# yassouali/pytorch-segmentation

Measured on NVIDIA H100. Metric: images/sec DeepLabV3+/ResNet101 513x513 train step (fwd+CE+bwd+SGD), higher is better.
Workload: dtype bf16

## Files before the change

### pytorch-segmentation_b200/csrc/seg_conv_tc.cu

```cuda
#include <cuda.h>
#include <mutex>
#include <stdlib.h>
#include "seg_common.cuh"
#include "seg_ptx.cuh"
#include "seg_sync.cuh"

namespace seg {
namespace tc {

using namespace ptx;

constexpr int BM = 128;
constexpr int BK = 64;
constexpr int A_BYTES = BM * 128;
constexpr int KIND_KK = 0, KIND_KM = 1, KIND_MM = 2;
constexpr int NTHREADS = 384;
constexpr int NCONS = 256;
constexpr int MAXT = 49;

struct TcParams {
  CUtensorMap mapA;
  CUtensorMap mapB;
  int M;
  int Ncols;
  int taps;
  int kchunks;
  int stride;
  int lower_h, lower_w;
  int PQ, Q;
  int x_im2col;
  int brows_per_tap;
  short tap_wt[MAXT];
  short tap_oh[MAXT];
  short tap_ow[MAXT];
  void* out;
  long long ldo;
  int out_dtype;
  float beta;
  const float* bias;
  double* stats;
  unsigned* stat_ticket;
  SyncDesc sync;
  int out_strided, out_H, out_W, osy, osx, opy, opx;
  int kblocks_total, kblocks_per_split;
  float* dw;
  int dw_K, dw_C;
  float* ws;
};

template <int BN>
struct Cfg {
  static constexpr int B_BYTES = BN * 128;
  static constexpr int STAGE_BYTES = A_BYTES + B_BYTES;
  static constexpr int STAGES = BN == 64 ? 6 : (BN == 128 ? 5 : 4);
  static constexpr int STAT_BYTES = 2 * 2 * BN * 4;
  static constexpr int SMEM = STAGES * STAGE_BYTES + STAT_BYTES + 1024  + 256 ;
  static_assert(STAGES * STAGE_BYTES >= BM * BN * 4, "staging tile must fit in the pipeline ring");
  static_assert(SMEM <= 227 * 1024, "shared memory per block");
};

__device__ __forceinline__ void row_to_coords(int m, int PQ, int Q, int stride, int lower_h, int lower_w, int& n, int& h,
                                              int& w) {
  n = m / PQ;
  int rem = m - n * PQ;
  int pp = rem / Q;
  int qq = rem - pp * Q;
  h = lower_h + pp * stride;
  w = lower_w + qq * stride;
}

template <int BN, int TA, int TB>
__device__ __forceinline__ void wgmma_tile(float* acc, uint64_t adesc, uint64_t bdesc, uint32_t accumulate) {
  if constexpr (BN == 64) wgmma_m64n64k16<TA, TB>(acc, adesc, bdesc, accumulate);
  else if constexpr (BN == 128) wgmma_m64n128k16<TA, TB>(acc, adesc, bdesc, accumulate);
  else wgmma_m64n256k16<TA, TB>(acc, adesc, bdesc, accumulate);
}

__device__ __forceinline__ void consumer_sync() { asm volatile("bar.sync 1, 256;" ::: "memory"); }

template <int BN, int KIND>
__global__ void __launch_bounds__(NTHREADS, 1) conv_gemm_tc(const __grid_constant__ TcParams p) {
  using C = Cfg<BN>;
  constexpr int STAGES = C::STAGES;
  extern __shared__ uint8_t smem_raw[];
  const uint32_t raw_addr = smem_u32(smem_raw);
  const uint32_t smem0 = (raw_addr + 1023u) & ~1023u;
  uint8_t* smem_gen = smem_raw + (smem0 - raw_addr);
  float* stat_sm = reinterpret_cast<float*>(smem_gen + STAGES * C::STAGE_BYTES);
  const uint32_t bar0 = smem0 + STAGES * C::STAGE_BYTES + C::STAT_BYTES;
  auto full_bar = [&](int s) { return bar0 + 8u * s; };
  auto empty_bar = [&](int s) { return bar0 + 8u * (STAGES + s); };
  volatile int* flag_sm = reinterpret_cast<volatile int*>(smem_gen + STAGES * C::STAGE_BYTES + C::STAT_BYTES + 8 * 2 * STAGES);

  const int m0 = blockIdx.x * BM;
  const int n0 = blockIdx.y * BN;

  int tap_mm = 0, kb_begin = 0, kb_end = 0, num_iters;
  if (KIND == KIND_MM) {
    tap_mm = blockIdx.z % p.taps;
    const int split = blockIdx.z / p.taps;
    kb_begin = split * p.kblocks_per_split;
    kb_end = min(kb_begin + p.kblocks_per_split, p.kblocks_total);
    num_iters = max(kb_end - kb_begin, 0);
  } else {
    num_iters = p.taps * p.kchunks;
  }

  if (threadIdx.x == 0) {
    prefetch_tmap(&p.mapA);
    prefetch_tmap(&p.mapB);
    for (int s = 0; s < STAGES; ++s) {
      mbar_init(full_bar(s), 1);
      mbar_init(empty_bar(s), 8);
    }
    fence_mbar_init();
  }
  __syncthreads();
  pdl_wait();

  if (threadIdx.x < 128) {
    if (threadIdx.x == 0 && num_iters > 0) {
      if (KIND != KIND_MM) {
        int n_img = 0, h0 = 0, w0 = 0;
        if (p.x_im2col) row_to_coords(m0, p.PQ, p.Q, p.stride, p.lower_h, p.lower_w, n_img, h0, w0);
        int it = 0;
        for (int tap = 0; tap < p.taps; ++tap) {
          const int wtap = p.tap_wt[tap];
          const uint16_t oh = (uint16_t)p.tap_oh[tap], ow = (uint16_t)p.tap_ow[tap];
          for (int kc = 0; kc < p.kchunks; ++kc, ++it) {
            const int st = it % STAGES;
            const uint32_t ph = (it / STAGES) & 1;
            mbar_wait_nocall(empty_bar(st), ph ^ 1u);
            const uint32_t a_dst = smem0 + st * C::STAGE_BYTES;
            const uint32_t b_dst = a_dst + A_BYTES;
            mbar_arrive_expect_tx(full_bar(st), C::STAGE_BYTES);
            if (p.x_im2col)
              tma_load_im2col_4d(a_dst, &p.mapA, full_bar(st), kc * BK, w0, h0, n_img, ow, oh);
            else
              tma_load_2d(a_dst, &p.mapA, full_bar(st), kc * BK, m0);
            if (KIND == KIND_KK) {
              tma_load_2d(b_dst, &p.mapB, full_bar(st), kc * BK, wtap * p.brows_per_tap + n0);
            } else {
#pragma unroll
              for (int j = 0; j < BN / 64; ++j)
                tma_load_2d(b_dst + j * 8192, &p.mapB, full_bar(st), n0 + j * 64, wtap * p.brows_per_tap + kc * BK);
            }
          }
        }
      } else {
        const uint16_t oh = (uint16_t)p.tap_oh[tap_mm], ow = (uint16_t)p.tap_ow[tap_mm];
        int it = 0;
        for (int kb = kb_begin; kb < kb_end; ++kb, ++it) {
          const int st = it % STAGES;
          const uint32_t ph = (it / STAGES) & 1;
          mbar_wait_nocall(empty_bar(st), ph ^ 1u);
          const uint32_t a_dst = smem0 + st * C::STAGE_BYTES;
          const uint32_t b_dst = a_dst + A_BYTES;
          const int pix0 = kb * BK;
          mbar_arrive_expect_tx(full_bar(st), C::STAGE_BYTES);
          tma_load_2d(a_dst, &p.mapA, full_bar(st), m0, pix0);
          tma_load_2d(a_dst + 8192, &p.mapA, full_bar(st), m0 + 64, pix0);
          if (p.x_im2col) {
            int n_img, h0, w0;
            row_to_coords(pix0, p.PQ, p.Q, p.stride, p.lower_h, p.lower_w, n_img, h0, w0);
#pragma unroll
            for (int j = 0; j < BN / 64; ++j)
              tma_load_im2col_4d(b_dst + j * 8192, &p.mapB, full_bar(st), n0 + j * 64, w0, h0, n_img, ow, oh);
          } else {
#pragma unroll
            for (int j = 0; j < BN / 64; ++j) tma_load_2d(b_dst + j * 8192, &p.mapB, full_bar(st), n0 + j * 64, pix0);
          }
        }
      }
    }
    return;
  }

  if (KIND == KIND_MM && num_iters == 0) return;
  const int ctid = threadIdx.x - 128;
  const int cw = ctid >> 7;
  const int warp = (ctid >> 5) & 3, lane = ctid & 31;
  float acc[BN / 2];
#pragma unroll
  for (int i = 0; i < BN / 2; ++i) acc[i] = 0.f;
  {
    constexpr int TA = (KIND == KIND_MM) ? 1 : 0;
    constexpr int TB = (KIND == KIND_KK) ? 0 : 1;
    for (int it = 0; it < num_iters; ++it) {
      const int st = it % STAGES;
      mbar_wait_nocall(full_bar(st), (it / STAGES) & 1);
      const uint32_t a_addr = smem0 + st * C::STAGE_BYTES + cw * 8192;
      const uint32_t b_addr = smem0 + st * C::STAGE_BYTES + A_BYTES;
      const uint64_t adesc0 = make_smem_desc_sw128(a_addr, TA ? 8192 : 16, 1024);
      const uint64_t bdesc0 = make_smem_desc_sw128(b_addr, TB ? 8192 : 16, 1024);
      wgmma_fence();
#pragma unroll
      for (int k = 0; k < BK / 16; ++k) {
        const uint64_t adesc = adesc0 + (uint64_t)(TA ? (k * 2048 >> 4) : (k * 32 >> 4));
        const uint64_t bdesc = bdesc0 + (uint64_t)(TB ? (k * 2048 >> 4) : (k * 32 >> 4));
        wgmma_tile<BN, TA, TB>(acc, adesc, bdesc, 1u);
      }
      wgmma_commit();
      wgmma_wait<1>();
      __syncwarp();
      if (it > 0 && lane == 0) mbar_arrive(empty_bar((it - 1) % STAGES));
    }
    wgmma_wait<0>();
  }
  consumer_sync();

  const bool out_f32 = (KIND == KIND_MM) || p.out_dtype != SEG_DT_BF16;
  const int esize = out_f32 ? 4 : 2;
  const int CPR = BN * esize / 16;
  const int swz = (CPR >= 32 ? 31 : CPR - 1);
  uint8_t* stage = smem_gen;
  const int ncols_tile = min(BN, p.Ncols - n0);
  {
    const int r0 = cw * 64 + warp * 16 + (lane >> 2);
#pragma unroll
    for (int j = 0; j < BN / 8; ++j) {
      const int col = j * 8 + 2 * (lane & 3);
      float b0 = 0.f, b1 = 0.f;
      if (KIND != KIND_MM && p.bias) {
        if (col < ncols_tile) b0 = __ldg(p.bias + n0 + col);
        if (col + 1 < ncols_tile) b1 = __ldg(p.bias + n0 + col + 1);
      }
#pragma unroll
      for (int h = 0; h < 2; ++h) {
        const int r = r0 + 8 * h;
        const float x0 = acc[4 * j + 2 * h] + b0, x1 = acc[4 * j + 2 * h + 1] + b1;
        const int byte = col * esize;
        uint8_t* dst = stage + (size_t)r * (BN * esize) + ((((byte >> 4) ^ (r & swz))) << 4) + (byte & 15);
        if (out_f32)
          *reinterpret_cast<float2*>(dst) = make_float2(x0, x1);
        else
          *reinterpret_cast<__nv_bfloat162*>(dst) = __floats2bfloat162_rn(x0, x1);
      }
    }
  }
  consumer_sync();

  if (KIND == KIND_MM) {
    float* base = p.ws ? p.ws + (size_t)(blockIdx.z / p.taps) * p.taps * p.dw_K * p.dw_C : p.dw;
    for (int idx = ctid; idx < BM * CPR; idx += NCONS) {
      const int tr = idx / CPR, c16 = idx - tr * CPR;
      const int row = m0 + tr, col0 = c16 * 4;
      if (row >= p.M || col0 >= ncols_tile) continue;
      const float4 v = *reinterpret_cast<const float4*>(stage + (size_t)tr * (BN * 4) + ((c16 ^ (tr & swz)) << 4));
      float* dst = base + ((size_t)tap_mm * p.dw_K + row) * p.dw_C + n0 + col0;
      const bool vec = col0 + 4 <= ncols_tile && ((reinterpret_cast<uintptr_t>(dst) & 15) == 0);
      const float a[4] = {v.x, v.y, v.z, v.w};
      if (p.ws) {
        if (vec)
          *reinterpret_cast<float4*>(dst) = v;
        else
          for (int i = 0; i < 4; ++i)
            if (col0 + i < ncols_tile) dst[i] = a[i];
      } else if (vec) {
        asm volatile("red.global.add.v4.f32 [%0], {%1, %2, %3, %4};" ::"l"(dst), "f"(v.x), "f"(v.y), "f"(v.z), "f"(v.w)
                     : "memory");
      } else {
        for (int i = 0; i < 4; ++i)
          if (col0 + i < ncols_tile) atomicAdd(dst + i, a[i]);
      }
    }
    return;
  }

  if (p.stats) {
    constexpr int NG = NCONS / BN, RPG = BM / NG;
    const int c = ctid % BN, g = ctid / BN;
    const int rend = min((g + 1) * RPG, p.M - m0);
    float s1 = 0.f, s2 = 0.f;
    const int byte = c * esize;
    for (int r = g * RPG; r < rend; ++r) {
      const uint8_t* src = stage + (size_t)r * (BN * esize) + ((((byte >> 4) ^ (r & swz))) << 4) + (byte & 15);
      const float x = out_f32 ? *reinterpret_cast<const float*>(src) : bf2f(*reinterpret_cast<const __nv_bfloat16*>(src));
      s1 += x;
      s2 = fmaf(x, x, s2);
    }
    stat_sm[(g * 2 + 0) * BN + c] = s1;
    stat_sm[(g * 2 + 1) * BN + c] = s2;
  }

  {
    const int nchunks = (ncols_tile * esize + 15) >> 4;
    const bool vec_ok = ((p.ldo * esize) & 15) == 0 && ((reinterpret_cast<uintptr_t>(p.out) + (size_t)n0 * esize) & 15) == 0;
    for (int idx = ctid; idx < BM * CPR; idx += NCONS) {
      const int tr = idx / CPR;
      const int c16 = idx - tr * CPR;
      if (c16 >= nchunks) continue;
      const int grow = m0 + tr;
      if (grow >= p.M) continue;
      long long pixel = grow;
      if (p.out_strided) {
        const int n = grow / p.PQ;
        const int rem = grow - n * p.PQ;
        const int i = rem / p.Q, j = rem - i * p.Q;
        pixel = ((long long)n * p.out_H + (i * p.osy + p.opy)) * p.out_W + (j * p.osx + p.opx);
      }
      const uint8_t* src = stage + (size_t)tr * (BN * esize) + ((c16 ^ (tr & swz)) << 4);
      uint8_t* dst = reinterpret_cast<uint8_t*>(p.out) + ((size_t)pixel * p.ldo + n0) * esize + ((size_t)c16 << 4);
      const int first_col = (c16 << 4) / esize;
      const bool full = first_col + 16 / esize <= ncols_tile;
      if (!out_f32) {
        bf16x8 val = *reinterpret_cast<const bf16x8*>(src);
        if (vec_ok && full) {
          if (p.beta != 0.f) {
            float a[8], b[8];
            unpack8(val, a);
            unpack8(*reinterpret_cast<const bf16x8*>(dst), b);
#pragma unroll
            for (int k = 0; k < 8; ++k) a[k] += p.beta * b[k];
            val = pack8(a);
          }
          *reinterpret_cast<bf16x8*>(dst) = val;
        } else {
          float a[8];
          unpack8(val, a);
          __nv_bfloat16* d = reinterpret_cast<__nv_bfloat16*>(dst);
          for (int k = 0; k < 8; ++k)
            if (first_col + k < ncols_tile) {
              float o = a[k];
              if (p.beta != 0.f) o += p.beta * bf2f(d[k]);
              d[k] = f2bf(o);
            }
        }
      } else {
        const float4 val = *reinterpret_cast<const float4*>(src);
        const float a[4] = {val.x, val.y, val.z, val.w};
        float* d = reinterpret_cast<float*>(dst);
        if (vec_ok && full && p.beta == 0.f) {
          *reinterpret_cast<float4*>(d) = val;
        } else {
          for (int k = 0; k < 4; ++k)
            if (first_col + k < ncols_tile) d[k] = (p.beta != 0.f) ? a[k] + p.beta * d[k] : a[k];
        }
      }
    }
  }
  if (num_iters > 0 && ctid == 0) pdl_trigger();

  if (p.stats) {
    constexpr int NG = NCONS / BN;
    consumer_sync();
    for (int c = ctid; c < ncols_tile; c += NCONS) {
      float a = 0.f, b = 0.f;
#pragma unroll
      for (int g = 0; g < NG; ++g) {
        a += stat_sm[(g * 2 + 0) * BN + c];
        b += stat_sm[(g * 2 + 1) * BN + c];
      }
      atomicAdd(p.stats + n0 + c, (double)a);
      atomicAdd(p.stats + p.Ncols + n0 + c, (double)b);
    }
    if (p.sync.world > 0)
      sync_push_when_last<false>(p.sync, p.stats, 2 * p.Ncols, p.stat_ticket, gridDim.x * gridDim.y, ctid, NCONS,
                          [] { asm volatile("bar.sync 1, 256;" ::: "memory"); }, flag_sm);
  }
}

typedef CUresult (*EncodeTiledFn)(CUtensorMap*, CUtensorMapDataType, cuuint32_t, void*, const cuuint64_t*,
                                  const cuuint64_t*, const cuuint32_t*, const cuuint32_t*, CUtensorMapInterleave,
                                  CUtensorMapSwizzle, CUtensorMapL2promotion, CUtensorMapFloatOOBfill);
typedef CUresult (*EncodeIm2colFn)(CUtensorMap*, CUtensorMapDataType, cuuint32_t, void*, const cuuint64_t*,
                                   const cuuint64_t*, const int*, const int*, cuuint32_t, cuuint32_t,
                                   const cuuint32_t*, CUtensorMapInterleave, CUtensorMapSwizzle,
                                   CUtensorMapL2promotion, CUtensorMapFloatOOBfill);
static EncodeTiledFn g_encode_tiled = nullptr;
static EncodeIm2colFn g_encode_im2col = nullptr;
static int g_driver_version = 0;

static int resolve_driver() {
  static std::once_flag once;
  static int status = 0;
  std::call_once(once, [] {
    void* f1 = nullptr;
    void* f2 = nullptr;
    cudaDriverEntryPointQueryResult q;
    if (cudaGetDriverEntryPoint("cuTensorMapEncodeTiled", &f1, cudaEnableDefault, &q) != cudaSuccess || !f1) status = 1;
    if (cudaGetDriverEntryPoint("cuTensorMapEncodeIm2col", &f2, cudaEnableDefault, &q) != cudaSuccess || !f2) status = 1;
    g_encode_tiled = (EncodeTiledFn)f1;
    g_encode_im2col = (EncodeIm2colFn)f2;
    cudaDriverGetVersion(&g_driver_version);
  });
  if (status) set_error("cannot resolve cuTensorMapEncode* driver entry points");
  return status;
}

static int make_map_2d(CUtensorMap* m, const void* ptr, int64_t rows, int64_t cols, int64_t ld, int box_rows) {
  if (resolve_driver()) return 1;
  SEG_REQUIRE((reinterpret_cast<uintptr_t>(ptr) & 15) == 0, "TMA: base pointer not 16-byte aligned");
  SEG_REQUIRE(ld % 8 == 0, "TMA: row pitch %lld not a multiple of 8 elements", (long long)ld);
  cuuint64_t dims[2] = {(cuuint64_t)cols, (cuuint64_t)rows};
  cuuint64_t strides[1] = {(cuuint64_t)ld * 2};
  cuuint32_t box[2] = {64, (cuuint32_t)box_rows};
  cuuint32_t es[2] = {1, 1};
  CUresult r = g_encode_tiled(m, CU_TENSOR_MAP_DATA_TYPE_BFLOAT16, 2, const_cast<void*>(ptr), dims, strides, box, es,
                              CU_TENSOR_MAP_INTERLEAVE_NONE, CU_TENSOR_MAP_SWIZZLE_128B,
                              CU_TENSOR_MAP_L2_PROMOTION_L2_256B, CU_TENSOR_MAP_FLOAT_OOB_FILL_NONE);
  SEG_REQUIRE(r == CUDA_SUCCESS, "cuTensorMapEncodeTiled failed (%d) rows=%lld cols=%lld ld=%lld box_rows=%d", (int)r,
              (long long)rows, (long long)cols, (long long)ld, box_rows);
  return 0;
}

static int make_map_im2col(CUtensorMap* m, const void* ptr, int N, int H, int W, int C, int64_t ld, int lower_w,
                           int lower_h, int upper_w, int upper_h, int stride, int pixels) {
  if (resolve_driver()) return 1;
  SEG_REQUIRE((reinterpret_cast<uintptr_t>(ptr) & 15) == 0, "TMA: base pointer not 16-byte aligned");
  SEG_REQUIRE(ld % 8 == 0, "TMA: channel pitch %lld not a multiple of 8", (long long)ld);
  SEG_REQUIRE(lower_w >= -128 && upper_w >= -128 && lower_w <= 127 && upper_w <= 127 && lower_h >= -128 &&
                  upper_h >= -128 && lower_h <= 127 && upper_h <= 127,
              "im2col corner out of range");
  cuuint64_t dims[4] = {(cuuint64_t)C, (cuuint64_t)W, (cuuint64_t)H, (cuuint64_t)N};
  cuuint64_t strides[3] = {(cuuint64_t)ld * 2, (cuuint64_t)W * ld * 2, (cuuint64_t)H * W * ld * 2};
  int lo[2] = {lower_w, lower_h};
  int up[2] = {upper_w, upper_h};
  cuuint32_t es[4] = {1, (cuuint32_t)stride, (cuuint32_t)stride, 1};
  CUresult r = g_encode_im2col(m, CU_TENSOR_MAP_DATA_TYPE_BFLOAT16, 4, const_cast<void*>(ptr), dims, strides, lo, up,
                               64, (cuuint32_t)pixels, es, CU_TENSOR_MAP_INTERLEAVE_NONE, CU_TENSOR_MAP_SWIZZLE_128B,
                               CU_TENSOR_MAP_L2_PROMOTION_L2_256B, CU_TENSOR_MAP_FLOAT_OOB_FILL_NONE);
  SEG_REQUIRE(r == CUDA_SUCCESS,
              "cuTensorMapEncodeIm2col failed (%d) N=%d H=%d W=%d C=%d ld=%lld lo=(%d,%d) up=(%d,%d) s=%d", (int)r, N, H,
              W, C, (long long)ld, lower_w, lower_h, upper_w, upper_h, stride);
  if (g_driver_version <= 13010) {
    const uint64_t bytes = (uint64_t)N * H * W * ld * 2;
    if (bytes < 131072) reinterpret_cast<uint64_t*>(m)[1] &= ~(1ull << 21);
  }
  return 0;
}

template <int BN, int KIND>
static int launch_kernel(const TcParams& p, dim3 grid, cudaStream_t stream) {
  static bool attr_set = false;
  auto kfn = conv_gemm_tc<BN, KIND>;
  if (!attr_set) {
    cudaError_t e = cudaFuncSetAttribute(kfn, cudaFuncAttributeMaxDynamicSharedMemorySize, Cfg<BN>::SMEM);
    SEG_REQUIRE(e == cudaSuccess, "cudaFuncSetAttribute(smem=%d): %s", Cfg<BN>::SMEM, cudaGetErrorString(e));
    attr_set = true;
  }
  launch_pdl(kfn, grid, dim3(NTHREADS), (size_t)Cfg<BN>::SMEM, stream, p);
  return check_launch("conv_gemm_tc");
}

template <int KIND>
static int launch_bn(int bn, const TcParams& p, dim3 grid, cudaStream_t stream) {
  switch (bn) {
    case 64: return launch_kernel<64, KIND>(p, grid, stream);
    case 128: return launch_kernel<128, KIND>(p, grid, stream);
    case 256: return launch_kernel<256, KIND>(p, grid, stream);
  }
  set_error("bad BN %d", bn);
  return 1;
}

static int pick_bn(int ncols) {
  if (ncols <= 64) return 64;
  if (ncols < 256) return 128;
  const int waste = ceil_div(ncols, 256) * 256 - ncols;
  return waste < 128 ? 256 : 128;
}

bool supported(const seg_conv_desc* d) {
  if (d->C % 8 != 0 || d->ldx % 8 != 0) return false;
  if (d->R != d->S) return false;
  if (d->R * d->S > MAXT) return false;
  if (d->pad > 127 || d->dil * (d->R - 1) - d->pad > 127 || d->dil * (d->R - 1) - d->pad < -127) return false;
  if (d->stride > 8) return false;
  return true;
}

static bool is_pointwise(const seg_conv_desc* d) { return d->R == 1 && d->S == 1 && d->stride == 1 && d->pad == 0; }

int conv_fwd(const seg_conv_desc* d, const void* x, const void* w, void* y, int y_dtype, const float* bias, float beta,
             double* stats, unsigned* stat_ticket, const SyncDesc* sync, cudaStream_t stream) {
  SEG_REQUIRE(supported(d), "wgmma conv fwd: unsupported shape (C=%d ldx=%d R=%d pad=%d dil=%d)", d->C, d->ldx, d->R,
              d->pad, d->dil);
  TcParams p;
  memset(&p, 0, sizeof(p));
  const int64_t M = (int64_t)d->N * d->P * d->Q;
  SEG_REQUIRE(M < (1ll << 31), "M too large");
  p.M = (int)M;
  p.Ncols = d->K;
  p.taps = d->R * d->S;
  for (int t = 0; t < p.taps; ++t) {
    p.tap_wt[t] = (short)t;
    p.tap_oh[t] = (short)((t / d->S) * d->dil);
    p.tap_ow[t] = (short)((t % d->S) * d->dil);
  }
  p.kchunks = ceil_div(d->C, BK);
  p.stride = d->stride;
  p.lower_h = p.lower_w = -d->pad;
  p.PQ = d->P * d->Q;
  p.Q = d->Q;
  p.brows_per_tap = d->K;
  p.out = y;
  p.ldo = d->ldy;
  p.out_dtype = y_dtype;
  p.beta = beta;
  p.bias = bias;
  p.stats = stats;
  p.stat_ticket = stat_ticket;
  if (sync && stats) {
    SEG_REQUIRE(stat_ticket != nullptr, "conv fwd: SyncBN needs a zeroed ticket word");
    SEG_REQUIRE(4 * d->K <= sync->n_max, "conv fwd: 2*K = %d fp64 statistics exceed the SyncBN buffer (%d floats)", 2 * d->K, sync->n_max);
    p.sync = *sync;
  }
  const int64_t m_tiles = ceil_div64(M, BM);
  const int bn = pick_bn(d->K);
  if (is_pointwise(d)) {
    p.x_im2col = 0;
    if (make_map_2d(&p.mapA, x, M, d->C, d->ldx, BM)) return 1;
  } else {
    p.x_im2col = 1;
    const int upper = d->pad - (d->R - 1) * d->dil;
    if (make_map_im2col(&p.mapA, x, d->N, d->H, d->W, d->C, d->ldx, -d->pad, -d->pad, upper, upper, d->stride, BM)) return 1;
  }
  if (make_map_2d(&p.mapB, w, (int64_t)p.taps * d->K, d->C, d->C, bn)) return 1;
  dim3 grid((unsigned)m_tiles, (unsigned)ceil_div(d->K, bn), 1);
  return launch_bn<KIND_KK>(bn, p, grid, stream);
}

static int floordiv(int a, int b) { return (a >= 0) ? a / b : -((-a + b - 1) / b); }

int conv_dgrad(const seg_conv_desc* d, const void* dy, const void* w, void* dx, float beta, cudaStream_t stream) {
  SEG_REQUIRE(supported(d) && d->ldy % 8 == 0, "wgmma conv dgrad: unsupported shape (stride=%d K=%d ldy=%d)", d->stride,
              d->K, d->ldy);
  const int s = d->stride;
  const int bn = pick_bn(d->C);
  for (int py = 0; py < s; ++py) {
    for (int px = 0; px < s; ++px) {
      const int Hs = (d->H - py + s - 1) / s, Ws = (d->W - px + s - 1) / s;
      if (Hs <= 0 || Ws <= 0) continue;
      TcParams p;
      memset(&p, 0, sizeof(p));
      int rh[8], oh[8], nh = 0, rw[8], ow[8], nw = 0;
      for (int r = 0; r < d->R; ++r) {
        const int num = py + d->pad - r * d->dil;
        if (((num % s) + s) % s == 0) { rh[nh] = r; oh[nh] = floordiv(num, s); ++nh; }
      }
      for (int q = 0; q < d->S; ++q) {
        const int num = px + d->pad - q * d->dil;
        if (((num % s) + s) % s == 0) { rw[nw] = q; ow[nw] = floordiv(num, s); ++nw; }
      }
      int min_oh = 0, min_ow = 0;
      for (int i = 0; i < nh; ++i) min_oh = (i == 0) ? oh[i] : min(min_oh, oh[i]);
      for (int i = 0; i < nw; ++i) min_ow = (i == 0) ? ow[i] : min(min_ow, ow[i]);
      p.taps = nh * nw;
      for (int i = 0; i < nh; ++i)
        for (int j = 0; j < nw; ++j) {
          const int t = i * nw + j;
          p.tap_wt[t] = (short)(rh[i] * d->S + rw[j]);
          p.tap_oh[t] = (short)(oh[i] - min_oh);
          p.tap_ow[t] = (short)(ow[j] - min_ow);
        }
      const int64_t M = (int64_t)d->N * Hs * Ws;
      SEG_REQUIRE(M < (1ll << 31), "M too large");
      p.M = (int)M;
      p.Ncols = d->C;
      p.kchunks = ceil_div(d->K, BK);
      p.stride = 1;
      p.lower_h = min_oh;
      p.lower_w = min_ow;
      p.PQ = Hs * Ws;
      p.Q = Ws;
      p.brows_per_tap = d->K;
      p.out = dx;
      p.ldo = d->ldx;
      p.out_dtype = SEG_DT_BF16;
      p.beta = beta;
      if (s > 1) {
        p.out_strided = 1;
        p.out_H = d->H;
        p.out_W = d->W;
        p.osy = p.osx = s;
        p.opy = py;
        p.opx = px;
      }
      const int64_t m_tiles = ceil_div64(M, BM);
      if (p.taps > 0) {
        const bool plain = (s == 1 && is_pointwise(d));
        if (plain) {
          p.x_im2col = 0;
          if (make_map_2d(&p.mapA, dy, M, d->K, d->ldy, BM)) return 1;
        } else {
          p.x_im2col = 1;
          const int upper_h = Hs - d->P + min_oh, upper_w = Ws - d->Q + min_ow;
          if (make_map_im2col(&p.mapA, dy, d->N, d->P, d->Q, d->K, d->ldy, min_ow, min_oh, upper_w, upper_h, 1, BM)) return 1;
        }
        if (make_map_2d(&p.mapB, w, (int64_t)d->R * d->S * d->K, d->C, d->C, 64)) return 1;
      } else {
        if (beta != 0.f) continue;
        if (make_map_2d(&p.mapA, w, (int64_t)d->R * d->S * d->K, d->C, d->C, BM)) return 1;
        if (make_map_2d(&p.mapB, w, (int64_t)d->R * d->S * d->K, d->C, d->C, 64)) return 1;
      }
      dim3 grid((unsigned)m_tiles, (unsigned)ceil_div(d->C, bn), 1);
      if (launch_bn<KIND_KM>(bn, p, grid, stream)) return 1;
    }
  }
  return 0;
}

__global__ void wgrad_split_reduce_kernel(const float* __restrict__ ws, int splits, int64_t n, float* __restrict__ dw) {
  for (int64_t i = blockIdx.x * (int64_t)blockDim.x + threadIdx.x; i < n; i += (int64_t)gridDim.x * blockDim.x) {
    float acc = ws[i];
    for (int s = 1; s < splits; ++s) acc += ws[(size_t)s * n + i];
    dw[i] += acc;
  }
}

static void wgrad_plan(const seg_conv_desc* d, int& bn, int& splits, int& kblocks_per_split) {
  const bool wide = d->R * d->S >= 9 && d->C >= 256 && d->C % 256 == 0;
  bn = (d->C <= 64) ? 64 : (wide ? 256 : 128);
  const int kblocks_total = (int)ceil_div64((int64_t)d->N * d->P * d->Q, BK);
  const int tiles = ceil_div(d->K, BM) * ceil_div(d->C, bn) * d->R * d->S;
  splits = max(1, num_sms() / tiles);
  splits = min(splits, kblocks_total);
  splits = min(splits, 1024);
  kblocks_per_split = ceil_div(kblocks_total, splits);
  splits = ceil_div(kblocks_total, kblocks_per_split);
}

int64_t wgrad_workspace_floats(const seg_conv_desc* d) {
  if (!supported(d)) return 0;
  int bn, splits, kps;
  wgrad_plan(d, bn, splits, kps);
  return splits > 1 ? (int64_t)splits * d->R * d->S * d->K * d->C : 0;
}

int conv_wgrad(const seg_conv_desc* d, const void* dy, const void* x, float* dw, float* ws, cudaStream_t stream) {
  SEG_REQUIRE(supported(d) && d->ldy % 8 == 0, "wgmma conv wgrad: unsupported shape");
  TcParams p;
  memset(&p, 0, sizeof(p));
  const int64_t npix = (int64_t)d->N * d->P * d->Q;
  SEG_REQUIRE(npix < (1ll << 31), "too many pixels");
  p.M = d->K;
  p.Ncols = d->C;
  p.taps = d->R * d->S;
  for (int t = 0; t < p.taps; ++t) {
    p.tap_wt[t] = (short)t;
    p.tap_oh[t] = (short)((t / d->S) * d->dil);
    p.tap_ow[t] = (short)((t % d->S) * d->dil);
  }
  p.stride = d->stride;
  p.lower_h = p.lower_w = -d->pad;
  p.PQ = d->P * d->Q;
  p.Q = d->Q;
  p.dw = dw;
  p.dw_K = d->K;
  p.dw_C = d->C;
  p.kblocks_total = (int)ceil_div64(npix, BK);
  int bn, splits;
  wgrad_plan(d, bn, splits, p.kblocks_per_split);
  SEG_REQUIRE(splits == 1 || ws != nullptr, "wgmma conv wgrad: %d k-splits need the workspace (seg_conv2d_wgrad_workspace_floats)", splits);
  SEG_REQUIRE((int64_t)(splits - 1) * p.kblocks_per_split < p.kblocks_total, "wgmma conv wgrad: split %d has no k-blocks", splits - 1);
  if (splits > 1) p.ws = ws;
  if (make_map_2d(&p.mapA, dy, npix, d->K, d->ldy, 64)) return 1;
  if (is_pointwise(d)) {
    p.x_im2col = 0;
    if (make_map_2d(&p.mapB, x, npix, d->C, d->ldx, 64)) return 1;
  } else {
    p.x_im2col = 1;
    const int upper = d->pad - (d->R - 1) * d->dil;
    if (make_map_im2col(&p.mapB, x, d->N, d->H, d->W, d->C, d->ldx, -d->pad, -d->pad, upper, upper, d->stride, 64)) return 1;
  }
  SEG_REQUIRE((unsigned)(p.taps * splits) <= 65535u, "wgrad grid.z too large");
  dim3 grid((unsigned)ceil_div(d->K, BM), (unsigned)ceil_div(d->C, bn), (unsigned)(p.taps * splits));
  if (launch_bn<KIND_MM>(bn, p, grid, stream)) return 1;
  if (splits == 1) return 0;
  const int64_t n = (int64_t)p.taps * d->K * d->C;
  wgrad_split_reduce_kernel<<<(unsigned)std::min<int64_t>(ceil_div64(n, 256), (int64_t)num_sms() * 8), 256, 0, stream>>>(ws, splits, n, dw);
  return check_launch("wgrad_split_reduce");
}

}
}
```

Before: 296.6.

## Split conv GEMM into main wave plus narrower-tile tail launch to cut wave quantization

Adds a wave planner for BN=256 convolutions. It launches the full-wave portion of M tiles with the wide tile and the leftover M tiles in a second launch with a narrower BN, using a cost model of waves times per-tile cost plus a launch gap. Batch-stat bookkeeping is made runtime-parameterized (rows per group, ticket total, M tile offset) so both launches share the stats and the SyncBN ticket. Dgrad also picks BN=64 when few k-blocks exist, and BN=64 stages drop from 6 to 4. The costs are a second kernel launch, a heuristic cost model, and unrolled stat loops becoming runtime loops.

```diff
diff --git a/pytorch-segmentation_b200/csrc/seg_conv_tc.cu b/pytorch-segmentation_b200/csrc/seg_conv_tc.cu
--- a/pytorch-segmentation_b200/csrc/seg_conv_tc.cu
+++ b/pytorch-segmentation_b200/csrc/seg_conv_tc.cu
@@ -39,8 +39,11 @@
   float beta;
   const float* bias;
   double* stats;
+  int stat_rpg;
   unsigned* stat_ticket;
+  unsigned ticket_total;
   SyncDesc sync;
+  int m_tile0;
   int out_strided, out_H, out_W, osy, osx, opy, opx;
   int kblocks_total, kblocks_per_split;
   float* dw;
@@ -52,8 +55,8 @@
 struct Cfg {
   static constexpr int B_BYTES = BN * 128;
   static constexpr int STAGE_BYTES = A_BYTES + B_BYTES;
-  static constexpr int STAGES = BN == 64 ? 6 : (BN == 128 ? 5 : 4);
-  static constexpr int STAT_BYTES = 2 * 2 * BN * 4;
+  static constexpr int STAGES = BN == 128 ? 5 : 4;
+  static constexpr int STAT_BYTES = (NCONS / BN) * 2 * BN * 4;
   static constexpr int SMEM = STAGES * STAGE_BYTES + STAT_BYTES + 1024  + 256 ;
   static_assert(STAGES * STAGE_BYTES >= BM * BN * 4, "staging tile must fit in the pipeline ring");
   static_assert(SMEM <= 227 * 1024, "shared memory per block");
@@ -92,7 +95,7 @@
   auto empty_bar = [&](int s) { return bar0 + 8u * (STAGES + s); };
   volatile int* flag_sm = reinterpret_cast<volatile int*>(smem_gen + STAGES * C::STAGE_BYTES + C::STAT_BYTES + 8 * 2 * STAGES);
 
-  const int m0 = blockIdx.x * BM;
+  const int m0 = (p.m_tile0 + blockIdx.x) * BM;
   const int n0 = blockIdx.y * BN;
 
   int tap_mm = 0, kb_begin = 0, kb_end = 0, num_iters;
@@ -267,20 +270,22 @@
     return;
   }
 
+  const int stat_ng = p.stats ? BM / p.stat_rpg : 0;
   if (p.stats) {
-    constexpr int NG = NCONS / BN, RPG = BM / NG;
     const int c = ctid % BN, g = ctid / BN;
-    const int rend = min((g + 1) * RPG, p.M - m0);
-    float s1 = 0.f, s2 = 0.f;
-    const int byte = c * esize;
-    for (int r = g * RPG; r < rend; ++r) {
-      const uint8_t* src = stage + (size_t)r * (BN * esize) + ((((byte >> 4) ^ (r & swz))) << 4) + (byte & 15);
-      const float x = out_f32 ? *reinterpret_cast<const float*>(src) : bf2f(*reinterpret_cast<const __nv_bfloat16*>(src));
-      s1 += x;
-      s2 = fmaf(x, x, s2);
-    }
-    stat_sm[(g * 2 + 0) * BN + c] = s1;
-    stat_sm[(g * 2 + 1) * BN + c] = s2;
+    if (g < stat_ng) {
+      const int rend = min((g + 1) * p.stat_rpg, p.M - m0);
+      float s1 = 0.f, s2 = 0.f;
+      const int byte = c * esize;
+      for (int r = g * p.stat_rpg; r < rend; ++r) {
+        const uint8_t* src = stage + (size_t)r * (BN * esize) + ((((byte >> 4) ^ (r & swz))) << 4) + (byte & 15);
+        const float x = out_f32 ? *reinterpret_cast<const float*>(src) : bf2f(*reinterpret_cast<const __nv_bfloat16*>(src));
+        s1 += x;
+        s2 = fmaf(x, x, s2);
+      }
+      stat_sm[(g * 2 + 0) * BN + c] = s1;
+      stat_sm[(g * 2 + 1) * BN + c] = s2;
+    }
   }
 
   {
@@ -342,12 +347,10 @@
   if (num_iters > 0 && ctid == 0) pdl_trigger();
 
   if (p.stats) {
-    constexpr int NG = NCONS / BN;
     consumer_sync();
     for (int c = ctid; c < ncols_tile; c += NCONS) {
       float a = 0.f, b = 0.f;
-#pragma unroll
-      for (int g = 0; g < NG; ++g) {
+      for (int g = 0; g < stat_ng; ++g) {
         a += stat_sm[(g * 2 + 0) * BN + c];
         b += stat_sm[(g * 2 + 1) * BN + c];
       }
@@ -355,7 +358,7 @@
       atomicAdd(p.stats + p.Ncols + n0 + c, (double)b);
     }
     if (p.sync.world > 0)
-      sync_push_when_last<false>(p.sync, p.stats, 2 * p.Ncols, p.stat_ticket, gridDim.x * gridDim.y, ctid, NCONS,
+      sync_push_when_last<false>(p.sync, p.stats, 2 * p.Ncols, p.stat_ticket, p.ticket_total, ctid, NCONS,
                           [] { asm volatile("bar.sync 1, 256;" ::: "memory"); }, flag_sm);
   }
 }
@@ -461,6 +464,50 @@
   return waste < 128 ? 256 : 128;
 }
 
+static float tile_cost(int bn) { return bn == 64 ? 0.60f : (bn == 128 ? 0.75f : 1.f); }
+constexpr float LAUNCH_GAP = 4.f;
+
+struct WavePlan {
+  int bn, n_tiles;
+  int m_main;
+  int bn_tail, n_tiles_tail;
+};
+
+static WavePlan plan_waves(int m_tiles, int ncols, int kblocks, int bn) {
+  WavePlan pl{bn, 0, m_tiles, 0, 0};
+  pl.n_tiles = ceil_div(ncols, pl.bn);
+  const int sms = num_sms();
+  const int m_main = (int)((int64_t)m_tiles * pl.n_tiles / sms * sms / pl.n_tiles);
+  if (pl.bn != 256 || m_main == 0 || m_main == m_tiles) return pl;
+  auto waves = [&](int64_t ctas) { return (float)ceil_div64(ctas, sms); };
+  float best = waves((int64_t)m_tiles * pl.n_tiles) * tile_cost(pl.bn) * kblocks;
+  for (int bt = 64; bt < pl.bn; bt *= 2) {
+    const int nt = ceil_div(ncols, bt);
+    const float t = (waves((int64_t)m_main * pl.n_tiles) * tile_cost(pl.bn) + waves((int64_t)(m_tiles - m_main) * nt) * tile_cost(bt)) *
+                        kblocks + LAUNCH_GAP;
+    if (t < best) {
+      best = t;
+      pl.m_main = m_main;
+      pl.bn_tail = bt;
+      pl.n_tiles_tail = nt;
+    }
+  }
+  return pl;
+}
+
+template <int KIND>
+static int launch_plan(const WavePlan& pl, int m_tiles, TcParams& p, const CUtensorMap* tail_mapB, cudaStream_t stream) {
+  p.stat_rpg = BM * pl.bn / NCONS;
+  p.ticket_total = (unsigned)(pl.m_main * pl.n_tiles + (m_tiles - pl.m_main) * pl.n_tiles_tail);
+  p.m_tile0 = 0;
+  if (launch_bn<KIND>(pl.bn, p, dim3((unsigned)pl.m_main, (unsigned)pl.n_tiles, 1), stream)) return 1;
+  if (pl.m_main == m_tiles) return 0;
+  TcParams q = p;
+  q.m_tile0 = pl.m_main;
+  if (tail_mapB) q.mapB = *tail_mapB;
+  return launch_bn<KIND>(pl.bn_tail, q, dim3((unsigned)(m_tiles - pl.m_main), (unsigned)pl.n_tiles_tail, 1), stream);
+}
+
 bool supported(const seg_conv_desc* d) {
   if (d->C % 8 != 0 || d->ldx % 8 != 0) return false;
   if (d->R != d->S) return false;
@@ -506,8 +553,8 @@
     SEG_REQUIRE(4 * d->K <= sync->n_max, "conv fwd: 2*K = %d fp64 statistics exceed the SyncBN buffer (%d floats)", 2 * d->K, sync->n_max);
     p.sync = *sync;
   }
-  const int64_t m_tiles = ceil_div64(M, BM);
-  const int bn = pick_bn(d->K);
+  const int m_tiles = (int)ceil_div64(M, BM);
+  const WavePlan pl = plan_waves(m_tiles, d->K, p.taps * p.kchunks, pick_bn(d->K));
   if (is_pointwise(d)) {
     p.x_im2col = 0;
     if (make_map_2d(&p.mapA, x, M, d->C, d->ldx, BM)) return 1;
@@ -516,9 +563,10 @@
     const int upper = d->pad - (d->R - 1) * d->dil;
     if (make_map_im2col(&p.mapA, x, d->N, d->H, d->W, d->C, d->ldx, -d->pad, -d->pad, upper, upper, d->stride, BM)) return 1;
   }
-  if (make_map_2d(&p.mapB, w, (int64_t)p.taps * d->K, d->C, d->C, bn)) return 1;
-  dim3 grid((unsigned)m_tiles, (unsigned)ceil_div(d->K, bn), 1);
-  return launch_bn<KIND_KK>(bn, p, grid, stream);
+  if (make_map_2d(&p.mapB, w, (int64_t)p.taps * d->K, d->C, d->C, pl.bn)) return 1;
+  CUtensorMap tail_mapB;
+  if (pl.m_main < m_tiles && make_map_2d(&tail_mapB, w, (int64_t)p.taps * d->K, d->C, d->C, pl.bn_tail)) return 1;
+  return launch_plan<KIND_KK>(pl, m_tiles, p, &tail_mapB, stream);
 }
 
 static int floordiv(int a, int b) { return (a >= 0) ? a / b : -((-a + b - 1) / b); }
@@ -527,7 +575,6 @@
   SEG_REQUIRE(supported(d) && d->ldy % 8 == 0, "wgmma conv dgrad: unsupported shape (stride=%d K=%d ldy=%d)", d->stride,
               d->K, d->ldy);
   const int s = d->stride;
-  const int bn = pick_bn(d->C);
   for (int py = 0; py < s; ++py) {
     for (int px = 0; px < s; ++px) {
       const int Hs = (d->H - py + s - 1) / s, Ws = (d->W - px + s - 1) / s;
@@ -577,7 +624,7 @@
         p.opy = py;
         p.opx = px;
       }
-      const int64_t m_tiles = ceil_div64(M, BM);
+      const int m_tiles = (int)ceil_div64(M, BM);
       if (p.taps > 0) {
         const bool plain = (s == 1 && is_pointwise(d));
         if (plain) {
@@ -594,8 +641,9 @@
         if (make_map_2d(&p.mapA, w, (int64_t)d->R * d->S * d->K, d->C, d->C, BM)) return 1;
         if (make_map_2d(&p.mapB, w, (int64_t)d->R * d->S * d->K, d->C, d->C, 64)) return 1;
       }
-      dim3 grid((unsigned)m_tiles, (unsigned)ceil_div(d->C, bn), 1);
-      if (launch_bn<KIND_KM>(bn, p, grid, stream)) return 1;
+      const int kblocks = p.taps * p.kchunks;
+      const WavePlan pl = plan_waves(m_tiles, d->C, kblocks, kblocks <= 4 ? 64 : pick_bn(d->C));
+      if (launch_plan<KIND_KM>(pl, m_tiles, p, nullptr, stream)) return 1;
     }
   }
   return 0;
```

Result: faster. 308.0, median of 6 (+3.8%).
